# tal-amir/fsw-gnn

Hardware: AMD Instinct MI355X
Metric: edges*slices/sec FSW_conv forward, 1M-node/10M-edge, 256 slices (higher is better)
Workload: dtype f32; 1 GPU; BASELINE config 3: ER multigraph 1000000 nodes / 10000000 edges (9999936 after coalesce), 128 feat, 256 slices, FSW_conv(128->128, embed_dim=257), full forward incl. CSR build and Linear layer; nodes=1000000, edges=10000000, edges_coalesced=9999936, slices=256, features=128, parallelism=single GPU

## Files before the change

fsw_gnn_amd/csrc/conv_fused.hip:

```cpp
#include <stdlib.h>
#include <algorithm>
#include "fsw_common.h"
#include "sortnet.h"
#include "row_pipeline.h"
#include "embed_cart.h"
#ifndef FSW_FUSED_PIPE_BARRIER
#define FSW_FUSED_PIPE_BARRIER 0
#endif

#ifndef FSW_FUSED_STAMPS
#define FSW_FUSED_STAMPS 0
#endif

namespace fsw {

#if FSW_FUSED_STAMPS
constexpr int kFusedStampWgs = 40000;
__device__ unsigned long long g_fused_stamps[kFusedStampWgs][4][8];
#define FSW_FSTAMP(i)                                                                      \
  do {                                                                                     \
    const unsigned long long now_ = clock64();                                             \
    if (lane_id() == 0 && blockIdx.x < kFusedStampWgs) g_fused_stamps[blockIdx.x][wave_id()][i] = now_ - fst_last; \
    fst_last = now_;                                                                       \
  } while (0)
#else
#define FSW_FSTAMP(i) do { } while (0)
#endif

using f32x16 = __attribute__((ext_vector_type(16))) float;

constexpr int kFusedRows = 32;
constexpr int kLdT = 132;
#ifndef FSW_FUSED_PREFETCH
#define FSW_FUSED_PREFETCH 8
#endif
#ifndef FSW_FUSED_NARROW_WAVES
#define FSW_FUSED_NARROW_WAVES 4
#endif

struct FusedArgs {
  const int32_t* rowptr;
  const int32_t* col;
  const int32_t* perm;
  const int32_t* bin_start;
  const float* Xp;
  int64_t ldp;
  int S;
  const float* table;
  int64_t ldt;
  const float* bias;
  float out_scale;
  int has_mass, mass_fn;
  float mass_scale;
  const float* Wq;
  int64_t ldw;
  const float* lin_bias;
  const float* Yin;
  int64_t ldyin;
  int yin_by_node;
  int Hout;
  int act;
  float slope;
  float* Y;
  int64_t ldy;
  int ldh;
  int tile_floats;
  int Kp;
};

template <int D, int RPW>
__device__ __forceinline__ void fused_embed_rows(const FusedArgs& a, int p, int nrows, float* __restrict__ H, int chunk) {
  constexpr int LPR = kWave / RPW;
  const int lane = lane_id();
  const int sub = RPW == 1 ? 0 : lane / LPR;
  const int k = chunk * kWave + (RPW == 1 ? lane : lane % LPR);
  const bool kvalid = k < a.S;
  const int kc = kvalid ? k : a.S - 1;
  const float b = a.bias ? a.out_scale * a.bias[a.has_mass + kc] : 0.f;
  if constexpr (D == 0) {
    for (int r = sub; r < nrows; r += RPW)
      if (kvalid) H[r * a.ldh + a.has_mass + k] = b;
  } else {
    float coef[D];
    const float* tab = a.table + (int64_t)(D * (D - 1) / 2) * a.ldt + kc;
#pragma unroll
    for (int t = 0; t < D; ++t) coef[t] = a.out_scale * tab[(int64_t)t * a.ldt];
    const int startv = a.rowptr[a.perm[p + min(lane, nrows - 1)]];
    float* hk = H + a.has_mass + kc;
    const int ldh = a.ldh;
    const int nsteps = (nrows + RPW - 1) / RPW;
    pipelined_rows<D, pipeline_depth<D>(), FSW_FUSED_PIPE_BARRIER>(
        nsteps, a.col, a.Xp + kc, a.ldp,
        [&](int r) {
          if constexpr (RPW == 1) return __builtin_amdgcn_readlane(startv, r);
          else return __shfl(startv, min(r * RPW + sub, nrows - 1));
        },
        [&](KeyNet<D>& net, int r) {
          sort_network<D>(net);
          float acc = b;
#pragma unroll
          for (int t = 0; t < D; ++t) acc = fmaf(coef[t], net.k[t], acc);
          const int row = RPW == 1 ? r : min(r * RPW + sub, nrows - 1);
          hk[row * ldh] = acc;
        });
  }
}

#define FSW_CASES_0_32(X)                                                                                                   \
  X(0) X(1) X(2) X(3) X(4) X(5) X(6) X(7) X(8) X(9) X(10) X(11) X(12) X(13) X(14) X(15) X(16) X(17) X(18) X(19) X(20) X(21) \
  X(22) X(23) X(24) X(25) X(26) X(27) X(28) X(29) X(30) X(31) X(32)

template <int ABL>
__device__ __forceinline__ void slab_mma(const FusedArgs& a, const float* __restrict__ H, int slab, int fr, int fh, f32x16& acc) {
  constexpr int kPrefetch = FSW_FUSED_PREFETCH;
  const int ngroups = a.Kp >> 3;
  const int j = min(slab * 32 + fr, (int)a.ldw - 1);
#pragma unroll
  for (int r = 0; r < 16; ++r) acc[r] = 0.f;
  const float* hp = H + fr * a.ldh + fh;
  const float4* wq = reinterpret_cast<const float4*>(a.Wq) + ((int64_t)j * 2 + fh);
  const int64_t gstride = a.ldw * 2;
  auto mma4 = [&](const float* h, const float4& bq) {
    if constexpr (ABL & 1) { asm volatile("" ::"v"(bq.x), "v"(bq.y), "v"(bq.z), "v"(bq.w)); return; }
    acc = __builtin_amdgcn_mfma_f32_32x32x2f32(h[0], bq.x, acc, 0, 0, 0);
    acc = __builtin_amdgcn_mfma_f32_32x32x2f32(h[2], bq.y, acc, 0, 0, 0);
    acc = __builtin_amdgcn_mfma_f32_32x32x2f32(h[4], bq.z, acc, 0, 0, 0);
    acc = __builtin_amdgcn_mfma_f32_32x32x2f32(h[6], bq.w, acc, 0, 0, 0);
  };
  float4 bq[kPrefetch];
#pragma unroll
  for (int u = 0; u < kPrefetch; ++u) bq[u] = wq[u * gstride];
  wq += kPrefetch * gstride;
  int g0 = 0;
  for (; g0 + kPrefetch <= ngroups; g0 += kPrefetch) {
#pragma unroll
    for (int u = 0; u < kPrefetch; ++u) {
      mma4(hp + 8 * (g0 + u), bq[u]);
      bq[u] = wq[u * gstride];
    }
    wq += kPrefetch * gstride;
  }
#pragma unroll
  for (int u = 0; u < kPrefetch; ++u)
    if (g0 + u < ngroups) mma4(hp + 8 * (g0 + u), bq[u]);
}

template <int TR>
__device__ __forceinline__ void fused_tile_init(const FusedArgs& a, int D, int p, int nrows, int K, float* H, int* nodeS) {
  if (threadIdx.x < TR) {
    const int r = threadIdx.x;
    for (int c = (r < nrows ? K : 0); c < a.ldh; ++c) H[r * a.ldh + c] = 0.f;
    nodeS[r] = r < nrows ? a.perm[p + r] : -1;
    if (a.has_mass && r < nrows)
      H[r * a.ldh] = mass_column((float)D, a.mass_fn, a.mass_scale, a.bias, a.out_scale);
  }
}

template <int DLO, int DHI, int WAVES_PER_SIMD, int ABL = 0, int RPW = 1, int TR = 32>
__global__ void __launch_bounds__(256, WAVES_PER_SIMD) k_conv_fused_unit(const FusedArgs a) {
  static_assert(TR == kFusedRows || (TR == 128 && RPW == 2), "tile rows");
  extern __shared__ __attribute__((aligned(16))) float smem[];
  float* H = smem;
  int* nodeS = reinterpret_cast<int*>(smem + a.tile_floats);

#if FSW_FUSED_STAMPS
  unsigned long long fst_last = clock64();
#endif
  int D, p = 0, pe = 0;
  if (!find_degree_tile<TR>(a.bin_start, DLO, DHI, (int)blockIdx.x, D, p, pe)) return;
  const int nrows = pe - p;
  const int wv = wave_id();
  const int lane = lane_id();
  const int K = a.has_mass + a.S;
  const int fr = lane & 31, fh = lane >> 5;

  fused_tile_init<TR>(a, D, p, nrows, K, H, nodeS);
  FSW_FSTAMP(0);
  const int nchunks = (a.S + kWave - 1) / kWave;
  const int ngroups = nchunks >= 3 ? 1 : 4 / nchunks;
  const int grows = TR / ngroups;
  for (int item = wv; item < nchunks * ngroups; item += 4) {
    const int chunk = item / ngroups, r0 = (item - chunk * ngroups) * grows;
    const int gn = min(nrows - r0, grows);
    if (gn <= 0) continue;
    switch (D) {
#define X(d)                                                  \
  case d:                                                     \
    if constexpr (d >= DLO && d <= DHI) fused_embed_rows<d, RPW>(a, p + r0, gn, H + r0 * a.ldh, chunk); \
    break;
      FSW_CASES_0_32(X)
#undef X
      default:
        break;
    }
  }
  FSW_FSTAMP(1);
#include "conv_fused_tail.inc"
}

struct FusedCartArgs {
  FusedArgs f;
  int slices, F;
  const float* ctable;
  int64_t ldct;
};

template <int D>
__device__ __forceinline__ void fused_cart_rows(const FusedCartArgs& a, int p, int nrows, float* H) {
  const FusedArgs& f_ = a.f;
  const int F = a.F, ldh = f_.ldh;
  if constexpr (D == 0) {
    const int W = a.slices * F;
    for (int i = threadIdx.x; i < nrows * W; i += blockDim.x) {
      const int r = i / W, c = i - r * W;
      H[r * ldh + f_.has_mass + c] = f_.bias ? f_.out_scale * f_.bias[f_.has_mass + c] : 0.f;
    }
  } else {
    ConstAS<float>* tab = as_const(a.ctable + (int64_t)(D * (D - 1) / 2) * a.ldct);
    const int items = nrows * a.slices;
    for (int i = threadIdx.x; i < items; i += blockDim.x) {
      const int r = i / a.slices, s = i - r * a.slices;
      const int start = f_.rowptr[f_.perm[p + r]];
      KeyNet<D> net;
#pragma unroll
      for (int t = 0; t < D; ++t) net.k[t] = f_.Xp[(int64_t)f_.col[start + t] * f_.ldp + s];
      sort_network<D>(net);
      const int c0 = f_.has_mass + s * F;
      float* h = H + r * ldh + c0;
      for (int f = 0; f < F; ++f) {
        float acc = f_.bias ? f_.bias[c0 + f] : 0.f;
#pragma unroll
        for (int t = 0; t < D; ++t) acc = fmaf(tab[(int64_t)t * a.ldct + f], net.k[t], acc);
        h[f] = f_.out_scale * acc;
      }
    }
  }
}

template <int WAVES_PER_SIMD>
__global__ void __launch_bounds__(256, WAVES_PER_SIMD) k_conv_fused_cart(const FusedCartArgs ca) {
  extern __shared__ __attribute__((aligned(16))) float smem[];
  float* H = smem;
  int* nodeS = reinterpret_cast<int*>(smem + ca.f.tile_floats);
  int D, p = 0, pe = 0;
  if (!find_degree_tile<kFusedRows>(ca.f.bin_start, 0, FSW_REG_MAX_DEG, (int)blockIdx.x, D, p, pe)) return;
  const int nrows = pe - p;
  const int wv = wave_id();
  const int lane = lane_id();
  fused_tile_init<kFusedRows>(ca.f, D, p, nrows, ca.f.has_mass + ca.f.S, H, nodeS);
  switch (D) {
#define X(d)                           \
  case d:                              \
    fused_cart_rows<d>(ca, p, nrows, H); \
    break;
    FSW_CASES_0_32(X)
#undef X
    default:
      break;
  }
#if FSW_FUSED_STAMPS
  unsigned long long fst_last = clock64();
#endif
  {
    const FusedArgs& a = ca.f;
    constexpr int ABL = 0, TR = kFusedRows;
    const int fr = lane & 31, fh = lane >> 5;
#include "conv_fused_tail.inc"
  }
}

__global__ void __launch_bounds__(256) k_pack_linear(const float* __restrict__ W, int64_t ldw_in, int Hout, int col0, int K,
                                                     float* __restrict__ Wq, int64_t ldwq, int64_t ngroups,
                                                     const float* __restrict__ W2, int d2, float* __restrict__ W2out, int64_t ldw2out) {
  const int64_t nq = ngroups * ldwq * 8;
  const int64_t total = nq + (W2out ? (int64_t)Hout * d2 : 0);
  for (int64_t idx = (int64_t)blockIdx.x * blockDim.x + threadIdx.x; idx < total; idx += (int64_t)gridDim.x * blockDim.x) {
    if (idx < nq) {
      const int e = (int)(idx & 7), h = e >> 2, i = e & 3;
      const int64_t gj = idx >> 3;
      const int64_t g = gj / ldwq, j = gj - g * ldwq;
      const int64_t k = 8 * g + 2 * i + h;
      Wq[idx] = (j < Hout && k < K) ? W[j * ldw_in + col0 + k] : 0.f;
    } else {
      const int64_t t = idx - nq;
      const int64_t j = t / d2, c = t - j * d2;
      W2out[j * ldw2out + c] = W2[j * ldw_in + c];
    }
  }
}

__global__ void __launch_bounds__(256) k_add_bias_act(float* __restrict__ R, int64_t ldr, const float* __restrict__ Yin, int64_t ldyin,
                                                      const float* __restrict__ bias, int64_t rows, int H, int act, float slope) {
// ... 9 lines not shown
        float y = R[r * ldr + c + u];
        if (Yin) y += Yin[r * ldyin + c + u];
        if (bias) y += bias[c + u];
        if (act == 1) y = fmaxf(y, 0.f);
        else if (act == 2) y = y >= 0.f ? y : slope * y;
        v[u] = y;
      }
    }
#pragma unroll
    for (int u = 0; u < 4; ++u)
      if (c + u < H) R[r * ldr + c + u] = v[u];
  }
}

}

using namespace fsw;

extern "C" int fsw_add_bias_act_f32(float* R, int64_t ldr, const float* Yin, int64_t ldyin, const float* bias, int64_t rows, int H,
                                    int act, float slope, fsw_stream_t stream_) {
  hipStream_t stream = reinterpret_cast<hipStream_t>(stream_);
  if (rows == 0) return 0;
  FSW_REQUIRE(R && rows > 0 && H >= 1 && ldr >= H && (!Yin || ldyin >= H), "fsw_add_bias_act_f32: bad arguments");
  FSW_REQUIRE(act >= 0 && act <= 2, "fsw_add_bias_act_f32: act must be 0 (none), 1 (relu) or 2 (leaky relu)");
  const int64_t total = rows * ((H + 3) / 4);
  k_add_bias_act<<<(unsigned)std::min<int64_t>(ceil_div(total, 256), 4096), 256, 0, stream>>>(R, ldr, Yin, ldyin, bias, rows, H, act, slope);
  FSW_LAUNCH_CHECK();
  return 0;
}

extern "C" size_t fsw_packed_linear_floats(int K, int Hout) {
  return (size_t)(((K + 7) / 8) + 16) * (size_t)(((Hout + 31) / 32) * 32) * 8;
}

extern "C" int fsw_pack_linear_f32(const float* W, int64_t ldw_in, int Hout, int col0, int K, float* Wq, const float* W2, int d2,
                                   float* W2out, int64_t ldw2out, fsw_stream_t stream_) {
  hipStream_t stream = reinterpret_cast<hipStream_t>(stream_);
  FSW_REQUIRE(W && Wq && Hout >= 1 && K >= 1 && col0 >= 0 && ldw_in >= col0 + K, "fsw_pack_linear_f32: bad arguments");
  FSW_REQUIRE(((uintptr_t)Wq & 15) == 0, "fsw_pack_linear_f32: Wq must be 16-byte aligned");
  FSW_REQUIRE(!W2out || (W2 && d2 >= 1 && ldw2out >= d2), "fsw_pack_linear_f32: bad W2 block");
  const int64_t ldwq = ((Hout + 31) / 32) * 32, ngroups = (K + 7) / 8 + 16;
  const int64_t total = ngroups * ldwq * 8 + (W2out ? (int64_t)Hout * d2 : 0);
  k_pack_linear<<<(unsigned)std::min<int64_t>(ceil_div(total, 256), 2048), 256, 0, stream>>>(W, ldw_in, Hout, col0, K, Wq, ldwq, ngroups, W2,
                                                                                            d2, W2out, ldw2out);
  FSW_LAUNCH_CHECK();
  return 0;
}

#ifndef FSW_FUSED_NARROW_ROWS
#define FSW_FUSED_NARROW_ROWS 128
#endif
static bool fused_wide_tile(int S, int Hout) { return FSW_FUSED_NARROW_ROWS == 128 && S <= kWave / 2 && Hout <= 128; }

extern "C" size_t fsw_conv_fused_lds_bytes(int S, int has_mass) {
  const int Kp = (has_mass + S + 7) & ~7;
  const int ldh = Kp | 1;
  if (fused_wide_tile(S, 128))
    return (size_t)128 * ldh * sizeof(float) + 128 * sizeof(int) + (size_t)kFusedRows * kLdT * sizeof(float);
  return (size_t)kFusedRows * (ldh > kLdT ? ldh : kLdT) * sizeof(float) + kFusedRows * sizeof(int);
}

extern "C" int fsw_conv_fused_f32(const fsw_embed_args* args, const float* Wq, int64_t ldw, const float* lin_bias, int Hout,
                                  const float* Yin, int64_t ldyin, int yin_by_node, int act, float slope, float* Y, int64_t ldy,
                                  fsw_stream_t stream_) {
  hipStream_t stream = reinterpret_cast<hipStream_t>(stream_);
  FSW_REQUIRE(args && Wq && Y, "fsw_conv_fused_f32: null pointer");
  const fsw_embed_args& e = *args;
  FSW_REQUIRE(e.rowptr && e.col && e.perm && e.bin_start && e.Xp && e.unit_table, "fsw_conv_fused_f32: null pointer in args");
  FSW_REQUIRE(e.w == nullptr && e.tau <= 1.f, "fsw_conv_fused_f32: unit weights with tau <= 1 only");
  FSW_REQUIRE(e.S >= 1 && e.ldp >= e.S && e.ldt >= e.S && (e.has_mass == 0 || e.has_mass == 1), "fsw_conv_fused_f32: bad sizes");
  FSW_REQUIRE(!Yin || ldyin >= Hout, "fsw_conv_fused_f32: bad Yin stride");
  FSW_REQUIRE(Hout >= 1 && ldy >= Hout && ldw >= ((Hout + 31) / 32) * 32 && ldw % 32 == 0, "fsw_conv_fused_f32: bad output sizes");
  FSW_REQUIRE(((uintptr_t)Wq & 15) == 0, "fsw_conv_fused_f32: Wq must be 16-byte aligned");
  FSW_REQUIRE(act >= 0 && act <= 2, "fsw_conv_fused_f32: act must be 0 (none), 1 (relu) or 2 (leaky relu)");
  const bool wide_tile = fused_wide_tile(e.S, Hout);
  const size_t lds = wide_tile ? fsw_conv_fused_lds_bytes(e.S, e.has_mass)
                               : (size_t)kFusedRows * ((((e.has_mass + e.S + 7) & ~7) | 1) > kLdT ? (((e.has_mass + e.S + 7) & ~7) | 1) : kLdT) * sizeof(float) + kFusedRows * sizeof(int);
  FSW_REQUIRE(lds <= 64 * 1024, "fsw_conv_fused_f32: embed_dim too wide for the fused tile (%zu B of LDS)", lds);
  FusedArgs a;
  a.rowptr = e.rowptr; a.col = e.col; a.perm = e.perm; a.bin_start = e.bin_start;
  a.Xp = e.Xp; a.ldp = e.ldp; a.S = e.S; a.table = e.unit_table; a.ldt = e.ldt;
  a.bias = e.bias; a.out_scale = e.out_scale; a.has_mass = e.has_mass; a.mass_fn = e.mass_fn; a.mass_scale = e.mass_scale;
  a.Wq = Wq; a.ldw = ldw; a.lin_bias = lin_bias; a.Yin = Yin; a.ldyin = ldyin; a.yin_by_node = yin_by_node ? 1 : 0; a.Hout = Hout; a.act = act; a.slope = slope;
  a.Y = Y; a.ldy = ldy;
  a.Kp = (e.has_mass + e.S + 7) & ~7;
  a.ldh = a.Kp | 1;
  a.tile_floats = wide_tile ? 128 * a.ldh : kFusedRows * (a.ldh > kLdT ? a.ldh : kLdT);
  const int64_t nblocks = ceil_div(e.num_rows, kFusedRows) + FSW_REG_MAX_DEG + 1;
#ifdef FSW_ABLATION
  const char* abl_env = getenv("FSW_FUSED_ABL");
  const int abl = abl_env ? atoi(abl_env) : 0;
#define FSW_ABL_CASE(v)                                                                   \
  if (abl == v) {                                                                         \
    k_conv_fused_unit<0, FSW_REG_MAX_DEG, 4, v><<<(unsigned)nblocks, 256, lds, stream>>>(a); \
    FSW_LAUNCH_CHECK();                                                                   \
    return 0;                                                                             \
  }
  FSW_ABL_CASE(1) FSW_ABL_CASE(2) FSW_ABL_CASE(4) FSW_ABL_CASE(6) FSW_ABL_CASE(7)
#endif
  if (wide_tile) {
    const int64_t nb128 = ceil_div(e.num_rows, 128) + FSW_REG_MAX_DEG + 1;
    k_conv_fused_unit<0, FSW_REG_MAX_DEG, FSW_FUSED_NARROW_WAVES, 0, 2, 128><<<(unsigned)nb128, 256, lds, stream>>>(a);
  } else if (e.S <= kWave / 2)
    k_conv_fused_unit<0, FSW_REG_MAX_DEG, FSW_FUSED_NARROW_WAVES, 0, 2><<<(unsigned)nblocks, 256, lds, stream>>>(a);
  else
    k_conv_fused_unit<0, FSW_REG_MAX_DEG, 4><<<(unsigned)nblocks, 256, lds, stream>>>(a);
  FSW_LAUNCH_CHECK();
  return 0;
}

static size_t fused_tile_bytes(int K) {
  const int ldh = ((K + 7) & ~7) | 1;
  return (size_t)kFusedRows * (ldh > kLdT ? ldh : kLdT) * sizeof(float) + kFusedRows * sizeof(int);
}

extern "C" size_t fsw_conv_fused_cart_lds_bytes(int S, int F, int has_mass) {
  const int64_t K = (int64_t)has_mass + (int64_t)S * F;
  return K > (1 << 20) ? (size_t)-1 : fused_tile_bytes((int)K);
}

extern "C" int fsw_conv_fused_cart_f32(const fsw_cart_args* c, const float* Wq, int64_t ldw, const float* lin_bias, int Hout,
                                       const float* Yin, int64_t ldyin, int yin_by_node, int act, float slope, float* Y, int64_t ldy,
                                       fsw_stream_t stream_) {
  hipStream_t stream = reinterpret_cast<hipStream_t>(stream_);
  int rc;
  if ((rc = cart_check_common(c))) return rc;
  FSW_REQUIRE(Wq && Y, "fsw_conv_fused_cart_f32: null pointer");
  FSW_REQUIRE(c->value_dtype == 0 && !c->g, "fsw_conv_fused_cart_f32: float32 forward only");
  FSW_REQUIRE(c->perm && c->bin_start && c->bin_start_host, "fsw_conv_fused_cart_f32: needs perm, bin_start and its host copy");
  FSW_REQUIRE(c->w == nullptr && c->tau <= 1.0, "fsw_conv_fused_cart_f32: unit weights with tau <= 1 only");
  FSW_REQUIRE(c->unit_table && c->ldt >= c->F, "fsw_conv_fused_cart_f32: needs the unit coefficient table of the F frequencies");
  FSW_REQUIRE(!Yin || ldyin >= Hout, "fsw_conv_fused_cart_f32: bad Yin stride");
  FSW_REQUIRE(Hout >= 1 && ldy >= Hout && ldw >= ((Hout + 31) / 32) * 32 && ldw % 32 == 0, "fsw_conv_fused_cart_f32: bad output sizes");
  FSW_REQUIRE(((uintptr_t)Wq & 15) == 0, "fsw_conv_fused_cart_f32: Wq must be 16-byte aligned");
  FSW_REQUIRE(act >= 0 && act <= 2, "fsw_conv_fused_cart_f32: act must be 0 (none), 1 (relu) or 2 (leaky relu)");
  const size_t lds = fsw_conv_fused_cart_lds_bytes(c->S, c->F, c->has_mass);
  FSW_REQUIRE(lds <= 64 * 1024, "fsw_conv_fused_cart_f32: S * F too wide for the fused tile (%zu B of LDS)", lds);
  const int32_t* bs = c->bin_start_host;
  FSW_REQUIRE(bs[FSW_NUM_BINS] == bs[FSW_BIN_MID0], "fsw_conv_fused_cart_f32: rows of at most %d neighbours only", FSW_REG_MAX_DEG);
  FSW_REQUIRE(bs[FSW_BIN_MID0] - bs[0] == c->num_rows, "fsw_conv_fused_cart_f32: bin table does not cover num_rows");
  int64_t tiles = 0;
  for (int d = 0; d <= FSW_REG_MAX_DEG; ++d) tiles += ceil_div(bs[d + 1] - bs[d], kFusedRows);
  if (tiles == 0) return 0;
  FusedCartArgs a;
  FusedArgs& f = a.f;
  f.rowptr = c->rowptr; f.col = c->col; f.perm = c->perm; f.bin_start = c->bin_start;
  f.Xp = (const float*)c->Xp; f.ldp = c->ldp; f.S = c->S * c->F; f.table = nullptr; f.ldt = 0;
  f.bias = (const float*)c->bias; f.out_scale = (float)c->out_scale; f.has_mass = c->has_mass; f.mass_fn = c->mass_fn;
  f.mass_scale = (float)c->mass_scale;
  f.Wq = Wq; f.ldw = ldw; f.lin_bias = lin_bias; f.Yin = Yin; f.ldyin = ldyin; f.yin_by_node = yin_by_node ? 1 : 0; f.Hout = Hout;
  f.act = act; f.slope = slope; f.Y = Y; f.ldy = ldy;
  f.Kp = (c->has_mass + f.S + 7) & ~7;
  f.ldh = f.Kp | 1;
  f.tile_floats = kFusedRows * (f.ldh > kLdT ? f.ldh : kLdT);
  a.slices = c->S; a.F = c->F; a.ctable = c->unit_table; a.ldct = c->ldt;
  k_conv_fused_cart<4><<<(unsigned)tiles, 256, lds, stream>>>(a);
  FSW_LAUNCH_CHECK();
  return 0;
}

#if FSW_FUSED_STAMPS
extern "C" int fsw_debug_fused_stamps(unsigned long long* out, int max_wgs) {
  FSW_CHECK_HIP(hipDeviceSynchronize());
  const int nw = max_wgs < fsw::kFusedStampWgs ? max_wgs : fsw::kFusedStampWgs;
  FSW_CHECK_HIP(hipMemcpyFromSymbol(out, HIP_SYMBOL(fsw::g_fused_stamps), sizeof(unsigned long long) * (size_t)nw * 4 * 8));
  return 0;
}
#endif
```

fsw_gnn_amd/csrc/conv_fused_tail.inc:

```
  const int nslabs = (a.Hout + 31) / 32;
  if (nslabs <= 4) {
    float lb[2];
#pragma unroll
    for (int h = 0; h < 2; ++h) lb[h] = (!a.Yin && a.lin_bias && lane + 64 * h < a.Hout) ? a.lin_bias[lane + 64 * h] : 0.f;
    float* T = TR == kFusedRows ? smem : reinterpret_cast<float*>(nodeS + TR);
#pragma unroll 1
    for (int r0 = 0; r0 < TR; r0 += kFusedRows) {
      if (TR > kFusedRows && r0 >= nrows) break;
      const int nsub = min(nrows - r0, kFusedRows);
      float yin[16];
#pragma unroll
      for (int q = 0; q < 16; ++q) yin[q] = 0.f;
      if ((ABL & 2) == 0 && a.Yin) {
#pragma unroll
        for (int q = 0; q < 16; ++q) {
          const int row = r0 + min(wv * 8 + (q >> 1), nsub - 1), c = min(lane + 64 * (q & 1), a.Hout - 1);
          yin[q] = a.Yin[(int64_t)(a.yin_by_node ? a.perm[p + row] : p + row) * a.ldyin + c];
        }
      }
      FSW_FSTAMP(2);
      __syncthreads();
      FSW_FSTAMP(3);
      f32x16 acc;
      if (wv < nslabs) slab_mma<ABL>(a, H + r0 * a.ldh, wv, fr, fh, acc);
      FSW_FSTAMP(4);
      if (TR == kFusedRows) __syncthreads();
      if (wv < nslabs) {
#pragma unroll
        for (int r = 0; r < 16; ++r) T[((r & 3) + 8 * (r >> 2) + 4 * fh) * kLdT + wv * 32 + fr] = acc[r];
      }
      __syncthreads();
      FSW_FSTAMP(5);
#pragma unroll
      for (int rr = 0; rr < 8; ++rr) {
        const int row = wv * 8 + rr;
        const int node = row < nsub ? nodeS[r0 + row] : -1;
        if (node < 0) continue;
#pragma unroll
        for (int h = 0; h < 2; ++h) {
          const int c = lane + 64 * h;
          if (c < a.Hout) {
            float y = T[row * kLdT + c] + lb[h] + yin[rr * 2 + h];
            if (a.act == 1) y = fmaxf(y, 0.f);
            else if (a.act == 2) y = y >= 0.f ? y : a.slope * y;
            if ((ABL & 4) == 0 || y == 12345.f) a.Y[(int64_t)node * a.ldy + c] = y;
          }
        }
      }
    }
    FSW_FSTAMP(6);
    return;
  }

  __syncthreads();
  for (int slab = wv; slab < nslabs; slab += 4) {
    const int j = slab * 32 + fr;
    float yin[16];
#pragma unroll
    for (int r = 0; r < 16; ++r) {
      const int row = (r & 3) + 8 * (r >> 2) + 4 * fh;
      yin[r] = (a.Yin && row < nrows && j < a.Hout) ? a.Yin[(int64_t)(a.yin_by_node ? a.perm[p + row] : p + row) * a.ldyin + j] : 0.f;
    }
    f32x16 acc;
    slab_mma<ABL>(a, H, slab, fr, fh, acc);
    if (j < a.Hout) {
      const float lb = (!a.Yin && a.lin_bias) ? a.lin_bias[j] : 0.f;
#pragma unroll
      for (int r = 0; r < 16; ++r) {
        const int node = nodeS[(r & 3) + 8 * (r >> 2) + 4 * fh];
        if (node >= 0) {
          float y = acc[r] + lb + yin[r];
          if (a.act == 1) y = fmaxf(y, 0.f);
          else if (a.act == 2) y = y >= 0.f ? y : a.slope * y;
          a.Y[(int64_t)node * a.ldy + j] = y;
        }
      }
    }
  }
```

fsw_gnn_amd/csrc/fsw_common.h:

```cpp
#pragma once
#include <stdlib.h>
#include <algorithm>
#include <hip/hip_runtime.h>
#include <stdint.h>
#include <stdio.h>
#include <atomic>
#include "../../include/fsw_hip.h"

namespace fsw {

void set_error(const char* fmt, ...);

#define FSW_CHECK_HIP(expr)                                                              \
  do {                                                                                   \
    hipError_t e_ = (expr);                                                              \
    if (e_ != hipSuccess) {                                                              \
      fsw::set_error("%s failed: %s (%s:%d)", #expr, hipGetErrorString(e_), __FILE__, __LINE__); \
      return 2;                                                                          \
    }                                                                                    \
  } while (0)

#define FSW_REQUIRE(cond, ...)            \
  do {                                    \
    if (!(cond)) {                        \
      fsw::set_error(__VA_ARGS__);        \
      return 1;                           \
    }                                     \
  } while (0)

#define FSW_LAUNCH_CHECK() FSW_CHECK_HIP(hipGetLastError())

struct PerDeviceOnce {
  std::atomic<bool> done[64];
};
#define FSW_SET_MAX_LDS_ONCE(kernel, bytes)                                                                          \
  do {                                                                                                               \
    static fsw::PerDeviceOnce once_;                                                                                 \
    int dev_ = 0;                                                                                                    \
    FSW_CHECK_HIP(hipGetDevice(&dev_));                                                                              \
    if (dev_ < 0 || dev_ >= 64 || !once_.done[dev_].load(std::memory_order_relaxed)) {                               \
      FSW_CHECK_HIP(hipFuncSetAttribute(reinterpret_cast<const void*>(kernel), hipFuncAttributeMaxDynamicSharedMemorySize, (int)(bytes))); \
      if (dev_ >= 0 && dev_ < 64) once_.done[dev_].store(true, std::memory_order_relaxed);                           \
    }                                                                                                                \
  } while (0)

constexpr int kWave = 64;

__host__ __device__ inline int64_t ceil_div(int64_t a, int64_t b) { return (a + b - 1) / b; }

__device__ __forceinline__ int lane_id() { return threadIdx.x & (kWave - 1); }
__device__ __forceinline__ int wave_id() { return __builtin_amdgcn_readfirstlane(threadIdx.x >> 6); }
__device__ __forceinline__ int uniform(int v) { return __builtin_amdgcn_readfirstlane(v); }

__host__ __device__ inline int degree_bin(int deg) {
  if (deg <= FSW_REG_MAX_DEG) return deg;
  if (deg > FSW_HUB_MAX_DEG) return FSW_BIN_GLOBAL;
  if (deg > FSW_LDS_MAX_DEG) return FSW_BIN_HUB0 + (deg > 4096) + (deg > 8192) + (deg > 16384);
  if (deg > FSW_MID_MAX_DEG) return FSW_BIN_LDS0 + (deg > 512) + (deg > 1024);
  constexpr int sizes[FSW_NUM_MID_BINS] = FSW_MID_SIZES;
  int i = 0;
#pragma unroll
  for (int j = 0; j < FSW_NUM_MID_BINS - 1; ++j) i += deg > sizes[j];
  return FSW_BIN_MID0 + i;
}

constexpr int kHubWMaxDeg = 8191;

inline int64_t bin_rows_or(const fsw_embed_args& a, int lo, int hi, int64_t upper) {
  return a.bin_start_host ? (int64_t)a.bin_start_host[hi + 1] - a.bin_start_host[lo] : upper;
}

__host__ __device__ inline uint32_t pow2ceil(uint32_t v) {
  uint32_t p = 1;
  while (p < v) p <<= 1;
  return p;
}

constexpr double kPi = 3.14159265358979323846;

__device__ __forceinline__ float mass_encode(float m, int fn) {
  if (fn == 1) return 2.f * (m / (sqrtf(m + 1.f) + 1.f));
  if (fn == 2) return log1pf(m);
  return m;
}
__device__ __forceinline__ double mass_encode(double m, int fn) {
  if (fn == 1) return 2.0 * (m / (sqrt(m + 1.0) + 1.0));
  if (fn == 2) return log1p(m);
  return m;
}
__device__ __forceinline__ float mass_column(float m, int mass_fn, float mass_scale, float b0, float out_scale) {
  return out_scale * (mass_encode(m, mass_fn) * mass_scale + b0);
}
__device__ __forceinline__ float mass_column(float m, int mass_fn, float mass_scale, const float* bias, float out_scale) {
  return out_scale * (mass_encode(m, mass_fn) * mass_scale + (bias ? bias[0] : 0.f));
}
template <class T>
__device__ __forceinline__ double mass_column(double m, int mass_fn, double mass_scale, const T* bias, double out_scale) {
  return out_scale * (mass_encode(m, mass_fn) * mass_scale + (bias ? (double)bias[0] : 0.0));
}

__device__ __forceinline__ float sin2pi_rev(double x) {
  const double r = x - rint(x);
  return sinpif(2.f * (float)r);
}

// ... 104 lines not shown
```

fsw_gnn_amd/csrc/project.hip:

```cpp
#include <stdlib.h>
#include <algorithm>
#include "fsw_common.h"

namespace fsw {

using f32x16 = __attribute__((ext_vector_type(16))) float;

constexpr int PBM = 128, PBN = 128, PBK = 32, PLD = PBK + 1;

template <bool VEC, class RowPtr>
__device__ __forceinline__ void stage_tile(RowPtr rowp, int k0, int kmax, float (*dst)[PLD], int& nonfinite,
                                           float* __restrict__ copy_dst, int64_t ld_copy, int64_t row0) {
  const int kq = (threadIdx.x & 7) * 4;
  const int r0 = threadIdx.x >> 3;
#pragma unroll
  for (int i = 0; i < 4; ++i) {
    const int r = r0 + 32 * i;
    const float* src = rowp(r);
    float v[4] = {0.f, 0.f, 0.f, 0.f};
    if (src) {
      const float* p = src + k0 + kq;
      if (VEC && k0 + kq + 3 < kmax) {
        float4 q = *reinterpret_cast<const float4*>(p);
        v[0] = q.x; v[1] = q.y; v[2] = q.z; v[3] = q.w;
      } else {
#pragma unroll
        for (int j = 0; j < 4; ++j)
          if (k0 + kq + j < kmax) v[j] = p[j];
      }
    }
#pragma unroll
    for (int j = 0; j < 4; ++j) {
      nonfinite |= !(fabsf(v[j]) <= 3.402823466e38f);
      dst[r][kq + j] = v[j];
      if (copy_dst && src && k0 + kq + j < kmax) copy_dst[(row0 + r) * ld_copy + k0 + kq + j] = v[j];
    }
  }
}

template <bool VEC>
__global__ void __launch_bounds__(256) k_project(const float* __restrict__ X, int64_t n, int d, int64_t ldx,
                                                 const float* __restrict__ V, int S, int64_t ldv, float* __restrict__ Xp,
                                                 int64_t ldp, int32_t* __restrict__ stats, int nct,
                                                 float* __restrict__ x_copy, int64_t ld_copy,
                                                 const float* __restrict__ W2, int H2, int64_t ldw2,
                                                 const float* __restrict__ b2, float* __restrict__ Y2, int64_t ldy2,
                                                 const int32_t* __restrict__ row_map) {
  __shared__ float As[PBM][PLD];
  __shared__ float Bs[PBN][PLD];
  const int ct = blockIdx.x % nct;
  const int64_t rt = blockIdx.x / nct;
  const int64_t row0 = rt * PBM;
  const int col0 = ct * PBN;
  const int lane = lane_id();
  const int wv = threadIdx.x >> 6;
  const int wr = wv >> 1, wc = wv & 1;
  const int fr = lane & 31, fh = lane >> 5;
  const int N = S + H2;

// ... 130 lines not shown
  int buf = 0;
  for (; tile < ntiles; tile += gridDim.x) {
    const int64_t next = tile + gridDim.x, next2 = next + gridDim.x;
    if (next < ntiles) store_tile(buf ^ 1, next, q0, q1);
    if (next2 < ntiles) load_tile(next2, q0, q1);
    f32x16 acc;
#pragma unroll
    for (int r = 0; r < 16; ++r) acc[r] = 0.f;
    const float* ap = &As[buf][fr][fh];
    if (slab_active) {
#pragma unroll
      for (int q = 0; q < KQ; ++q) acc = __builtin_amdgcn_mfma_f32_32x32x2f32(ap[2 * q], b[q], acc, 0, 0, 0);
    }
    if (dst) {
      const int64_t row0 = tile * BS_ROWS;
#pragma unroll
      for (int r = 0; r < 16; ++r) {
        const int64_t gr = row0 + (r & 3) + 8 * (r >> 2) + 4 * fh;
        if (gr < n) dst[((second && row_map) ? (int64_t)rmap[buf][(r & 3) + 8 * (r >> 2) + 4 * fh] : gr) * ldd] = acc[r] + add;
      }
    }
    __syncthreads();
    buf ^= 1;
  }
  if (stats && nonfinite) atomicOr(&stats[FSW_STAT_FLAGS], FSW_FLAG_X_NONFINITE);
}

typedef __bf16 bf16x8 __attribute__((ext_vector_type(8)));
typedef __bf16 bf16x4 __attribute__((ext_vector_type(4)));
#ifndef FSW_PROJECT_STAMPS
#define FSW_PROJECT_STAMPS 0
#endif
#if FSW_PROJECT_STAMPS
__device__ unsigned long long g_proj_stamps[1024][12][8];
#define FSW_STAMP(i)                                         \
  do {                                                       \
    const unsigned long long now_ = clock64();               \
    stamp_sum[i] += now_ - stamp_last;                       \
    stamp_last = now_;                                       \
  } while (0)
#else
#define FSW_STAMP(i) do { } while (0)
#endif
#ifndef FSW_PROJECT_ABL
#define FSW_PROJECT_ABL 0
#endif

__device__ __forceinline__ void split3(float v, __bf16& a, __bf16& b, __bf16& c) {
  a = (__bf16)v;
  const float r = v - (float)a;
  b = (__bf16)r;
  c = (__bf16)(r - (float)b);
}

template <int CTRL>
__device__ __forceinline__ float quad_perm(float v) {
  return __int_as_float(__builtin_amdgcn_mov_dpp(__float_as_int(v), CTRL, 0xF, 0xF, true));
}
__device__ __forceinline__ void quad_transpose(f32x16& acc, int lane) {
  const bool b0 = lane & 1, b1 = lane & 2;
#pragma unroll
  for (int s = 0; s < 4; s += 2)
#pragma unroll
    for (int j = 0; j < 4; ++j) {
      const float lo = acc[4 * s + j], hi = acc[4 * s + 4 + j];
      const float got = quad_perm<0xB1>(b0 ? lo : hi);
      acc[4 * s + j] = b0 ? got : lo;
      acc[4 * s + 4 + j] = b0 ? hi : got;
    }
#pragma unroll
  for (int s = 0; s < 2; ++s)
#pragma unroll
    for (int j = 0; j < 4; ++j) {
      const float lo = acc[4 * s + j], hi = acc[4 * s + 8 + j];
      const float got = quad_perm<0x4E>(b1 ? lo : hi);
      acc[4 * s + j] = b1 ? got : lo;
      acc[4 * s + 8 + j] = b1 ? hi : got;
    }
}
template <int K>
__device__ __forceinline__ int quad_bcast(int v) { return __builtin_amdgcn_mov_dpp(v, K * 0x55, 0xF, 0xF, true); }

template <int KS, bool FAST>
__global__ void __launch_bounds__(768) k_project_bf3(const float* __restrict__ X, int64_t n, int d, int64_t ldx,
                                                     const float* __restrict__ V, int S, int64_t ldv,
                                                     float* __restrict__ Xp, int64_t ldp, int32_t* __restrict__ stats,
                                                     float* __restrict__ x_copy, int64_t ld_copy,
                                                     const float* __restrict__ W2, int H2, int64_t ldw2,
                                                     const float* __restrict__ b2, float* __restrict__ Y2, int64_t ldy2,
                                                     const int32_t* __restrict__ row_map, int64_t ntiles, int nslab_waves,
                                                     int nsl1, int y2_vec) {
  static_assert(KS <= 8, "k_project_bf3: d <= 128");
  constexpr int B3_LD = 16 * KS + 8;
  constexpr int NQ = 3;
  extern __shared__ __attribute__((aligned(16))) char smem[];
  typedef __bf16 (*APlanes)[3][BS_ROWS][B3_LD];
  APlanes As = reinterpret_cast<APlanes>(smem);
  float* btab = reinterpret_cast<float*>(smem + sizeof(__bf16) * 2 * 3 * BS_ROWS * B3_LD);

  const int lane = lane_id();
  const int wv = __builtin_amdgcn_readfirstlane(threadIdx.x >> 6);
  const int fr = lane & 31, fh = lane >> 5;
  const int slab = blockIdx.y * nslab_waves + wv;
  const int nsl2 = (H2 + 31) >> 5;
  const bool slab_active = FAST || (wv < nslab_waves && slab < nsl1 + nsl2);
  const bool second = slab >= nsl1;
  const int c = second ? (slab - nsl1) * 32 + fr : slab * 32 + fr;
  const bool col_ok = slab_active && (second ? c < H2 : c < S);

  bf16x8 bw[3][KS];
  {
    const float* wrow = col_ok ? (second ? W2 + (int64_t)c * ldw2 : V + (int64_t)c * ldv) : nullptr;
#pragma unroll
    for (int s = 0; s < KS; ++s)
#pragma unroll
      for (int j = 0; j < 8; ++j) {
        const int k = 16 * s + 8 * fh + j;
        const float v = (wrow && k < d) ? wrow[k] : 0.f;
        __bf16 h1, h2, h3;
        split3(v, h1, h2, h3);
        bw[0][s][j] = h1;
        bw[1][s][j] = h2;
        bw[2][s][j] = h3;
      }
  }
  if (wv < nslab_waves && fh == 0) btab[wv * 32 + fr] = (col_ok && second && b2) ? b2[c] : 0.f;

  for (int i = threadIdx.x; i < 2 * 3 * BS_ROWS * B3_LD / 2; i += blockDim.x) reinterpret_cast<uint32_t*>(smem)[i] = 0u;
  __syncthreads();

  const int d4 = d >> 2;
  const int per_tile = BS_ROWS * d4;
  auto magic = [](int dv) { return dv > 0 ? (unsigned)(((1u << 20) + dv - 1) / dv) : 0u; };
  auto fdiv = [](int i, unsigned m) { return (int)(((unsigned)i * m) >> 20); };
// ... 538 lines not shown
```

Before: 899.8 billion edges*slices/sec.

## Write fused conv output directly from MFMA registers via quad transpose and float4 stores

```diff
diff --git a/fsw_gnn_amd/csrc/conv_fused.hip b/fsw_gnn_amd/csrc/conv_fused.hip
--- a/fsw_gnn_amd/csrc/conv_fused.hip
+++ b/fsw_gnn_amd/csrc/conv_fused.hip
@@ -27,10 +27,7 @@
 #define FSW_FSTAMP(i) do { } while (0)
 #endif
 
-using f32x16 = __attribute__((ext_vector_type(16))) float;
-
 constexpr int kFusedRows = 32;
-constexpr int kLdT = 132;
 #ifndef FSW_FUSED_PREFETCH
 #define FSW_FUSED_PREFETCH 8
 #endif
@@ -122,10 +119,10 @@
   const int64_t gstride = a.ldw * 2;
   auto mma4 = [&](const float* h, const float4& bq) {
     if constexpr (ABL & 1) { asm volatile("" ::"v"(bq.x), "v"(bq.y), "v"(bq.z), "v"(bq.w)); return; }
-    acc = __builtin_amdgcn_mfma_f32_32x32x2f32(h[0], bq.x, acc, 0, 0, 0);
-    acc = __builtin_amdgcn_mfma_f32_32x32x2f32(h[2], bq.y, acc, 0, 0, 0);
-    acc = __builtin_amdgcn_mfma_f32_32x32x2f32(h[4], bq.z, acc, 0, 0, 0);
-    acc = __builtin_amdgcn_mfma_f32_32x32x2f32(h[6], bq.w, acc, 0, 0, 0);
+    acc = __builtin_amdgcn_mfma_f32_32x32x2f32(bq.x, h[0], acc, 0, 0, 0);
+    acc = __builtin_amdgcn_mfma_f32_32x32x2f32(bq.y, h[2], acc, 0, 0, 0);
+    acc = __builtin_amdgcn_mfma_f32_32x32x2f32(bq.z, h[4], acc, 0, 0, 0);
+    acc = __builtin_amdgcn_mfma_f32_32x32x2f32(bq.w, h[6], acc, 0, 0, 0);
   };
   float4 bq[kPrefetch];
 #pragma unroll
@@ -156,7 +153,7 @@
   }
 }
 
-template <int DLO, int DHI, int WAVES_PER_SIMD, int ABL = 0, int RPW = 1, int TR = 32>
+template <int DLO, int DHI, int WAVES_PER_SIMD, bool FAST, int ABL = 0, int RPW = 1, int TR = 32>
 __global__ void __launch_bounds__(256, WAVES_PER_SIMD) k_conv_fused_unit(const FusedArgs a) {
   static_assert(TR == kFusedRows || (TR == 128 && RPW == 2), "tile rows");
   extern __shared__ __attribute__((aligned(16))) float smem[];
@@ -237,7 +234,7 @@
   }
 }
 
-template <int WAVES_PER_SIMD>
+template <int WAVES_PER_SIMD, bool FAST>
 __global__ void __launch_bounds__(256, WAVES_PER_SIMD) k_conv_fused_cart(const FusedCartArgs ca) {
   extern __shared__ __attribute__((aligned(16))) float smem[];
   float* H = smem;
@@ -353,12 +350,17 @@
 #endif
 static bool fused_wide_tile(int S, int Hout) { return FSW_FUSED_NARROW_ROWS == 128 && S <= kWave / 2 && Hout <= 128; }
 
+static size_t fused_tile_bytes(int K, int rows) {
+  const int ldh = ((K + 7) & ~7) | 1;
+  return (size_t)rows * ldh * sizeof(float) + rows * sizeof(int);
+}
+
+static bool fused_vector_io(const float* Y, int64_t ldy, const float* Yin, int64_t ldyin, int Hout) {
+  return Hout >= 32 && ((uintptr_t)Y & 15) == 0 && ldy % 4 == 0 && (!Yin || (((uintptr_t)Yin & 15) == 0 && ldyin % 4 == 0));
+}
+
 extern "C" size_t fsw_conv_fused_lds_bytes(int S, int has_mass) {
-  const int Kp = (has_mass + S + 7) & ~7;
-  const int ldh = Kp | 1;
-  if (fused_wide_tile(S, 128))
-    return (size_t)128 * ldh * sizeof(float) + 128 * sizeof(int) + (size_t)kFusedRows * kLdT * sizeof(float);
-  return (size_t)kFusedRows * (ldh > kLdT ? ldh : kLdT) * sizeof(float) + kFusedRows * sizeof(int);
+  return fused_tile_bytes(has_mass + S, fused_wide_tile(S, 128) ? 128 : kFusedRows);
 }
 
 extern "C" int fsw_conv_fused_f32(const fsw_embed_args* args, const float* Wq, int64_t ldw, const float* lin_bias, int Hout,
@@ -375,8 +377,7 @@
   FSW_REQUIRE(((uintptr_t)Wq & 15) == 0, "fsw_conv_fused_f32: Wq must be 16-byte aligned");
   FSW_REQUIRE(act >= 0 && act <= 2, "fsw_conv_fused_f32: act must be 0 (none), 1 (relu) or 2 (leaky relu)");
   const bool wide_tile = fused_wide_tile(e.S, Hout);
-  const size_t lds = wide_tile ? fsw_conv_fused_lds_bytes(e.S, e.has_mass)
-                               : (size_t)kFusedRows * ((((e.has_mass + e.S + 7) & ~7) | 1) > kLdT ? (((e.has_mass + e.S + 7) & ~7) | 1) : kLdT) * sizeof(float) + kFusedRows * sizeof(int);
+  const size_t lds = fused_tile_bytes(e.has_mass + e.S, wide_tile ? 128 : kFusedRows);
   FSW_REQUIRE(lds <= 64 * 1024, "fsw_conv_fused_f32: embed_dim too wide for the fused tile (%zu B of LDS)", lds);
   FusedArgs a;
   a.rowptr = e.rowptr; a.col = e.col; a.perm = e.perm; a.bin_start = e.bin_start;
@@ -386,14 +387,16 @@
   a.Y = Y; a.ldy = ldy;
   a.Kp = (e.has_mass + e.S + 7) & ~7;
   a.ldh = a.Kp | 1;
-  a.tile_floats = wide_tile ? 128 * a.ldh : kFusedRows * (a.ldh > kLdT ? a.ldh : kLdT);
+  a.tile_floats = (wide_tile ? 128 : kFusedRows) * a.ldh;
+  const bool fast = fused_vector_io(Y, ldy, Yin, ldyin, Hout);
   const int64_t nblocks = ceil_div(e.num_rows, kFusedRows) + FSW_REG_MAX_DEG + 1;
 #ifdef FSW_ABLATION
   const char* abl_env = getenv("FSW_FUSED_ABL");
   const int abl = abl_env ? atoi(abl_env) : 0;
 #define FSW_ABL_CASE(v)                                                                   \
   if (abl == v) {                                                                         \
-    k_conv_fused_unit<0, FSW_REG_MAX_DEG, 4, v><<<(unsigned)nblocks, 256, lds, stream>>>(a); \
+    if (fast) k_conv_fused_unit<0, FSW_REG_MAX_DEG, 4, true, v><<<(unsigned)nblocks, 256, lds, stream>>>(a);  \
+    else k_conv_fused_unit<0, FSW_REG_MAX_DEG, 4, false, v><<<(unsigned)nblocks, 256, lds, stream>>>(a);      \
     FSW_LAUNCH_CHECK();                                                                   \
     return 0;                                                                             \
   }
@@ -401,23 +404,22 @@
 #endif
   if (wide_tile) {
     const int64_t nb128 = ceil_div(e.num_rows, 128) + FSW_REG_MAX_DEG + 1;
-    k_conv_fused_unit<0, FSW_REG_MAX_DEG, FSW_FUSED_NARROW_WAVES, 0, 2, 128><<<(unsigned)nb128, 256, lds, stream>>>(a);
-  } else if (e.S <= kWave / 2)
-    k_conv_fused_unit<0, FSW_REG_MAX_DEG, FSW_FUSED_NARROW_WAVES, 0, 2><<<(unsigned)nblocks, 256, lds, stream>>>(a);
-  else
-    k_conv_fused_unit<0, FSW_REG_MAX_DEG, 4><<<(unsigned)nblocks, 256, lds, stream>>>(a);
+    if (fast) k_conv_fused_unit<0, FSW_REG_MAX_DEG, FSW_FUSED_NARROW_WAVES, true, 0, 2, 128><<<(unsigned)nb128, 256, lds, stream>>>(a);
+    else k_conv_fused_unit<0, FSW_REG_MAX_DEG, FSW_FUSED_NARROW_WAVES, false, 0, 2, 128><<<(unsigned)nb128, 256, lds, stream>>>(a);
+  } else if (e.S <= kWave / 2) {
+    if (fast) k_conv_fused_unit<0, FSW_REG_MAX_DEG, FSW_FUSED_NARROW_WAVES, true, 0, 2><<<(unsigned)nblocks, 256, lds, stream>>>(a);
+    else k_conv_fused_unit<0, FSW_REG_MAX_DEG, FSW_FUSED_NARROW_WAVES, false, 0, 2><<<(unsigned)nblocks, 256, lds, stream>>>(a);
+  } else {
+    if (fast) k_conv_fused_unit<0, FSW_REG_MAX_DEG, 4, true><<<(unsigned)nblocks, 256, lds, stream>>>(a);
+    else k_conv_fused_unit<0, FSW_REG_MAX_DEG, 4, false><<<(unsigned)nblocks, 256, lds, stream>>>(a);
+  }
   FSW_LAUNCH_CHECK();
   return 0;
 }
 
-static size_t fused_tile_bytes(int K) {
-  const int ldh = ((K + 7) & ~7) | 1;
-  return (size_t)kFusedRows * (ldh > kLdT ? ldh : kLdT) * sizeof(float) + kFusedRows * sizeof(int);
-}
-
 extern "C" size_t fsw_conv_fused_cart_lds_bytes(int S, int F, int has_mass) {
   const int64_t K = (int64_t)has_mass + (int64_t)S * F;
-  return K > (1 << 20) ? (size_t)-1 : fused_tile_bytes((int)K);
+  return K > (1 << 20) ? (size_t)-1 : std::max(fused_tile_bytes((int)K, kFusedRows), (size_t)kFusedRows * (132 * sizeof(float) + sizeof(int)));
 }
 
 extern "C" int fsw_conv_fused_cart_f32(const fsw_cart_args* c, const float* Wq, int64_t ldw, const float* lin_bias, int Hout,
@@ -435,7 +437,8 @@
   FSW_REQUIRE(Hout >= 1 && ldy >= Hout && ldw >= ((Hout + 31) / 32) * 32 && ldw % 32 == 0, "fsw_conv_fused_cart_f32: bad output sizes");
   FSW_REQUIRE(((uintptr_t)Wq & 15) == 0, "fsw_conv_fused_cart_f32: Wq must be 16-byte aligned");
   FSW_REQUIRE(act >= 0 && act <= 2, "fsw_conv_fused_cart_f32: act must be 0 (none), 1 (relu) or 2 (leaky relu)");
-  const size_t lds = fsw_conv_fused_cart_lds_bytes(c->S, c->F, c->has_mass);
+  FSW_REQUIRE(fsw_conv_fused_cart_lds_bytes(c->S, c->F, c->has_mass) != (size_t)-1, "fsw_conv_fused_cart_f32: S * F too wide for the fused tile (LDS)");
+  const size_t lds = fused_tile_bytes(c->has_mass + c->S * c->F, kFusedRows);
   FSW_REQUIRE(lds <= 64 * 1024, "fsw_conv_fused_cart_f32: S * F too wide for the fused tile (%zu B of LDS)", lds);
   const int32_t* bs = c->bin_start_host;
   FSW_REQUIRE(bs[FSW_NUM_BINS] == bs[FSW_BIN_MID0], "fsw_conv_fused_cart_f32: rows of at most %d neighbours only", FSW_REG_MAX_DEG);
@@ -453,9 +456,10 @@
   f.act = act; f.slope = slope; f.Y = Y; f.ldy = ldy;
   f.Kp = (c->has_mass + f.S + 7) & ~7;
   f.ldh = f.Kp | 1;
-  f.tile_floats = kFusedRows * (f.ldh > kLdT ? f.ldh : kLdT);
+  f.tile_floats = kFusedRows * f.ldh;
   a.slices = c->S; a.F = c->F; a.ctable = c->unit_table; a.ldct = c->ldt;
-  k_conv_fused_cart<4><<<(unsigned)tiles, 256, lds, stream>>>(a);
+  if (fused_vector_io(Y, ldy, Yin, ldyin, Hout)) k_conv_fused_cart<4, true><<<(unsigned)tiles, 256, lds, stream>>>(a);
+  else k_conv_fused_cart<4, false><<<(unsigned)tiles, 256, lds, stream>>>(a);
   FSW_LAUNCH_CHECK();
   return 0;
 }
diff --git a/fsw_gnn_amd/csrc/conv_fused_tail.inc b/fsw_gnn_amd/csrc/conv_fused_tail.inc
--- a/fsw_gnn_amd/csrc/conv_fused_tail.inc
+++ b/fsw_gnn_amd/csrc/conv_fused_tail.inc
@@ -1,79 +1,72 @@
   const int nslabs = (a.Hout + 31) / 32;
-  if (nslabs <= 4) {
-    float lb[2];
+  const int cq = 8 * (fr & 3) + 4 * fh;
+  auto load_yin = [&](int slab, int ynode, float4 (&yin)[4], float (&lb)[4]) {
+    const int c0 = slab * 32 + cq;
 #pragma unroll
-    for (int h = 0; h < 2; ++h) lb[h] = (!a.Yin && a.lin_bias && lane + 64 * h < a.Hout) ? a.lin_bias[lane + 64 * h] : 0.f;
-    float* T = TR == kFusedRows ? smem : reinterpret_cast<float*>(nodeS + TR);
-#pragma unroll 1
-    for (int r0 = 0; r0 < TR; r0 += kFusedRows) {
-      if (TR > kFusedRows && r0 >= nrows) break;
-      const int nsub = min(nrows - r0, kFusedRows);
-      float yin[16];
+    for (int j = 0; j < 4; ++j) lb[j] = (!a.Yin && a.lin_bias) ? a.lin_bias[min(c0 + j, a.Hout - 1)] : 0.f;
 #pragma unroll
-      for (int q = 0; q < 16; ++q) yin[q] = 0.f;
-      if ((ABL & 2) == 0 && a.Yin) {
+    for (int k = 0; k < 4; ++k) yin[k] = make_float4(0.f, 0.f, 0.f, 0.f);
+    if ((ABL & 2) == 0 && a.Yin) {
+      const int yrow[4] = {quad_bcast<0>(ynode), quad_bcast<1>(ynode), quad_bcast<2>(ynode), quad_bcast<3>(ynode)};
+      if (FAST && slab * 32 + 32 <= a.Hout) {
 #pragma unroll
-        for (int q = 0; q < 16; ++q) {
-          const int row = r0 + min(wv * 8 + (q >> 1), nsub - 1), c = min(lane + 64 * (q & 1), a.Hout - 1);
-          yin[q] = a.Yin[(int64_t)(a.yin_by_node ? a.perm[p + row] : p + row) * a.ldyin + c];
-        }
-      }
-      FSW_FSTAMP(2);
-      __syncthreads();
-      FSW_FSTAMP(3);
-      f32x16 acc;
-      if (wv < nslabs) slab_mma<ABL>(a, H + r0 * a.ldh, wv, fr, fh, acc);
-      FSW_FSTAMP(4);
-      if (TR == kFusedRows) __syncthreads();
-      if (wv < nslabs) {
+        for (int k = 0; k < 4; ++k) yin[k] = *reinterpret_cast<const float4*>(a.Yin + (int64_t)yrow[k] * a.ldyin + c0);
+      } else {
 #pragma unroll
-        for (int r = 0; r < 16; ++r) T[((r & 3) + 8 * (r >> 2) + 4 * fh) * kLdT + wv * 32 + fr] = acc[r];
-      }
-      __syncthreads();
-      FSW_FSTAMP(5);
-#pragma unroll
-      for (int rr = 0; rr < 8; ++rr) {
-        const int row = wv * 8 + rr;
-        const int node = row < nsub ? nodeS[r0 + row] : -1;
-        if (node < 0) continue;
-#pragma unroll
-        for (int h = 0; h < 2; ++h) {
-          const int c = lane + 64 * h;
-          if (c < a.Hout) {
-            float y = T[row * kLdT + c] + lb[h] + yin[rr * 2 + h];
-            if (a.act == 1) y = fmaxf(y, 0.f);
-            else if (a.act == 2) y = y >= 0.f ? y : a.slope * y;
-            if ((ABL & 4) == 0 || y == 12345.f) a.Y[(int64_t)node * a.ldy + c] = y;
-          }
+        for (int k = 0; k < 4; ++k) {
+          const float* yr = a.Yin + (int64_t)yrow[k] * a.ldyin;
+          yin[k] = make_float4(yr[min(c0, a.Hout - 1)], yr[min(c0 + 1, a.Hout - 1)], yr[min(c0 + 2, a.Hout - 1)], yr[min(c0 + 3, a.Hout - 1)]);
         }
       }
     }
-    FSW_FSTAMP(6);
-    return;
+  };
+  float4 yin[4];
+  float lb[4];
+  if (wv < nslabs) {
+    const int r = min(fr, min(nrows, kFusedRows) - 1);
+    load_yin(wv, a.yin_by_node ? a.perm[p + r] : p + r, yin, lb);
   }
-
+  FSW_FSTAMP(2);
   __syncthreads();
-  for (int slab = wv; slab < nslabs; slab += 4) {
-    const int j = slab * 32 + fr;
-    float yin[16];
+  FSW_FSTAMP(3);
+#pragma unroll 1
+  for (int r0 = 0; r0 < TR; r0 += kFusedRows) {
+    if (TR > kFusedRows && r0 >= nrows) break;
+    const int nsub = min(nrows - r0, kFusedRows);
+    const int node = nodeS[r0 + fr];
+    const int nodek[4] = {quad_bcast<0>(node), quad_bcast<1>(node), quad_bcast<2>(node), quad_bcast<3>(node)};
+#pragma unroll 1
+    for (int slab = wv; slab < nslabs; slab += 4) {
+      if (r0 > 0 || slab != wv) {
+        const int r = r0 + min(fr, nsub - 1);
+        load_yin(slab, a.yin_by_node ? nodeS[r] : p + r, yin, lb);
+      }
+      f32x16 acc;
+      slab_mma<ABL>(a, H + r0 * a.ldh, slab, fr, fh, acc);
+      FSW_FSTAMP(4);
+      quad_transpose(acc, lane);
+      const int c0 = slab * 32 + cq;
+      const bool vec = FAST && slab * 32 + 32 <= a.Hout;
 #pragma unroll
-    for (int r = 0; r < 16; ++r) {
-      const int row = (r & 3) + 8 * (r >> 2) + 4 * fh;
-      yin[r] = (a.Yin && row < nrows && j < a.Hout) ? a.Yin[(int64_t)(a.yin_by_node ? a.perm[p + row] : p + row) * a.ldyin + j] : 0.f;
-    }
-    f32x16 acc;
-    slab_mma<ABL>(a, H, slab, fr, fh, acc);
-    if (j < a.Hout) {
-      const float lb = (!a.Yin && a.lin_bias) ? a.lin_bias[j] : 0.f;
+      for (int k = 0; k < 4; ++k) {
+        const float yi[4] = {yin[k].x, yin[k].y, yin[k].z, yin[k].w};
+        float y[4];
 #pragma unroll
-      for (int r = 0; r < 16; ++r) {
-        const int node = nodeS[(r & 3) + 8 * (r >> 2) + 4 * fh];
-        if (node >= 0) {
-          float y = acc[r] + lb + yin[r];
-          if (a.act == 1) y = fmaxf(y, 0.f);
-          else if (a.act == 2) y = y >= 0.f ? y : a.slope * y;
-          a.Y[(int64_t)node * a.ldy + j] = y;
+        for (int j = 0; j < 4; ++j) {
+          y[j] = acc[4 * k + j] + lb[j] + yi[j];
+          if (a.act == 1) y[j] = fmaxf(y[j], 0.f);
+          else if (a.act == 2) y[j] = y[j] >= 0.f ? y[j] : a.slope * y[j];
+        }
+        if (nodek[k] < 0) continue;
+        float* yrow = a.Y + (int64_t)nodek[k] * a.ldy;
+        if (vec) {
+          if ((ABL & 4) == 0 || y[0] == 12345.f) *reinterpret_cast<float4*>(yrow + c0) = make_float4(y[0], y[1], y[2], y[3]);
+        } else {
+#pragma unroll
+          for (int j = 0; j < 4; ++j)
+            if (c0 + j < a.Hout && ((ABL & 4) == 0 || y[j] == 12345.f)) yrow[c0 + j] = y[j];
         }
       }
+      FSW_FSTAMP(5);
     }
   }
diff --git a/fsw_gnn_amd/csrc/fsw_common.h b/fsw_gnn_amd/csrc/fsw_common.h
--- a/fsw_gnn_amd/csrc/fsw_common.h
+++ b/fsw_gnn_amd/csrc/fsw_common.h
@@ -51,6 +51,35 @@
 __device__ __forceinline__ int lane_id() { return threadIdx.x & (kWave - 1); }
 __device__ __forceinline__ int wave_id() { return __builtin_amdgcn_readfirstlane(threadIdx.x >> 6); }
 __device__ __forceinline__ int uniform(int v) { return __builtin_amdgcn_readfirstlane(v); }
+
+using f32x16 = __attribute__((ext_vector_type(16))) float;
+template <int CTRL>
+__device__ __forceinline__ float quad_perm(float v) {
+  return __int_as_float(__builtin_amdgcn_mov_dpp(__float_as_int(v), CTRL, 0xF, 0xF, true));
+}
+__device__ __forceinline__ void quad_transpose(f32x16& acc, int lane) {
+  const bool b0 = lane & 1, b1 = lane & 2;
+#pragma unroll
+  for (int s = 0; s < 4; s += 2)
+#pragma unroll
+    for (int j = 0; j < 4; ++j) {
+      const float lo = acc[4 * s + j], hi = acc[4 * s + 4 + j];
+      const float got = quad_perm<0xB1>(b0 ? lo : hi);
+      acc[4 * s + j] = b0 ? got : lo;
+      acc[4 * s + 4 + j] = b0 ? hi : got;
+    }
+#pragma unroll
+  for (int s = 0; s < 2; ++s)
+#pragma unroll
+    for (int j = 0; j < 4; ++j) {
+      const float lo = acc[4 * s + j], hi = acc[4 * s + 8 + j];
+      const float got = quad_perm<0x4E>(b1 ? lo : hi);
+      acc[4 * s + j] = b1 ? got : lo;
+      acc[4 * s + 8 + j] = b1 ? hi : got;
+    }
+}
+template <int K>
+__device__ __forceinline__ int quad_bcast(int v) { return __builtin_amdgcn_mov_dpp(v, K * 0x55, 0xF, 0xF, true); }
 
 __host__ __device__ inline int degree_bin(int deg) {
   if (deg <= FSW_REG_MAX_DEG) return deg;
diff --git a/fsw_gnn_amd/csrc/project.hip b/fsw_gnn_amd/csrc/project.hip
--- a/fsw_gnn_amd/csrc/project.hip
+++ b/fsw_gnn_amd/csrc/project.hip
@@ -3,8 +3,6 @@
 #include "fsw_common.h"
 
 namespace fsw {
-
-using f32x16 = __attribute__((ext_vector_type(16))) float;
 
 constexpr int PBM = 128, PBN = 128, PBK = 32, PLD = PBK + 1;
 
@@ -241,34 +239,6 @@
   b = (__bf16)r;
   c = (__bf16)(r - (float)b);
 }
-
-template <int CTRL>
-__device__ __forceinline__ float quad_perm(float v) {
-  return __int_as_float(__builtin_amdgcn_mov_dpp(__float_as_int(v), CTRL, 0xF, 0xF, true));
-}
-__device__ __forceinline__ void quad_transpose(f32x16& acc, int lane) {
-  const bool b0 = lane & 1, b1 = lane & 2;
-#pragma unroll
-  for (int s = 0; s < 4; s += 2)
-#pragma unroll
-    for (int j = 0; j < 4; ++j) {
-      const float lo = acc[4 * s + j], hi = acc[4 * s + 4 + j];
-      const float got = quad_perm<0xB1>(b0 ? lo : hi);
-      acc[4 * s + j] = b0 ? got : lo;
-      acc[4 * s + 4 + j] = b0 ? hi : got;
-    }
-#pragma unroll
-  for (int s = 0; s < 2; ++s)
-#pragma unroll
-    for (int j = 0; j < 4; ++j) {
-      const float lo = acc[4 * s + j], hi = acc[4 * s + 8 + j];
-      const float got = quad_perm<0x4E>(b1 ? lo : hi);
-      acc[4 * s + j] = b1 ? got : lo;
-      acc[4 * s + 8 + j] = b1 ? hi : got;
-    }
-}
-template <int K>
-__device__ __forceinline__ int quad_bcast(int v) { return __builtin_amdgcn_mov_dpp(v, K * 0x55, 0xF, 0xF, true); }
 
 template <int KS, bool FAST>
 __global__ void __launch_bounds__(768) k_project_bf3(const float* __restrict__ X, int64_t n, int d, int64_t ldx,
```

Result: no change. 907.8 billion edges*slices/sec (median of 6 runs) (+0.9%).
